# illini-robomaster/irmv_detection

Measured on AMD Instinct MI355X. Metric: end-to-end FPS (preprocess→NMS→PnP) 640×640 YOLOv8n, 1/2/4/8 MI355X, higher is better.
Workload: dtype f16

## Files before the change

irmv_detection_amd/csrc/irmv_common.hpp:

```cpp
#pragma once

#include <hip/hip_runtime.h>

#include <cstdint>
#include <cstdlib>

namespace irmv {

typedef _Float16 half_t;
typedef _Float16 half8 __attribute__((ext_vector_type(8)));
typedef _Float16 half4 __attribute__((ext_vector_type(4)));
typedef float f32x4 __attribute__((ext_vector_type(4)));

constexpr float kActScale = 1.44269504088896341f;
constexpr float kActUnscale = 0.693147180559945309f;
typedef unsigned int u32x4_t __attribute__((ext_vector_type(4)));
__device__ __forceinline__ float silu_rcp(float y) { return __builtin_amdgcn_rcpf(1.0f + __builtin_amdgcn_exp2f(-y)); }
__device__ __forceinline__ unsigned int silu_pack2(float y0, float y1)
{
    const float r0 = silu_rcp(y0), r1 = silu_rcp(y1);
    unsigned int o;
    asm("v_fma_mixlo_f16 %0, %1, %2, 0" : "=v"(o) : "v"(y0), "v"(r0));
    asm("v_fma_mixhi_f16 %0, %1, %2, 0" : "+v"(o) : "v"(y1), "v"(r1));
    return o;
}
__device__ __forceinline__ half8 silu_pack8(float y0, float y1, float y2, float y3, float y4, float y5, float y6, float y7)
{
    return __builtin_bit_cast(half8, (u32x4_t){silu_pack2(y0, y1), silu_pack2(y2, y3), silu_pack2(y4, y5), silu_pack2(y6, y7)});
}
__device__ __forceinline__ half4 silu_pack4(float y0, float y1, float y2, float y3)
{
    typedef unsigned int u32x2_t __attribute__((ext_vector_type(2)));
    return __builtin_bit_cast(half4, (u32x2_t){silu_pack2(y0, y1), silu_pack2(y2, y3)});
}
__device__ __forceinline__ void mfma_operand_fence(half4 &x) { asm volatile("s_nop 1" : "+v"(x)); }
__device__ __forceinline__ void mfma_operand_fence(half8 &x, half8 &y) { asm volatile("s_nop 1" : "+v"(x), "+v"(y)); }
__device__ __forceinline__ half_t silu_add_res(float y, float res)
{
    float p = y * silu_rcp(y);
    asm("" : "+v"(p));
    float s = p + res;
    asm("" : "+v"(s));
    return (half_t)s;
}

__device__ __forceinline__ void tile_image(int id, int tiles, int batch, int xcd, int &tile, int &image)
{
    const int full = xcd ? (batch >> 3) * 8 * tiles : 0;
    if (id < full) {
        const int j = id >> 3;
        image = (j / tiles) * 8 + (id & 7);
        tile = j % tiles;
    } else {
        const int r = id - full;
        image = (full / tiles) + r / tiles;
        tile = r % tiles;
    }
}

inline int xcd_image_order()
{
    const char *v = getenv("IRMV_XCD_IMAGES");
    return (v && v[0] == '0') ? 0 : 1;
}

inline int wres_stagger()
{
    const char *v = getenv("IRMV_WRES_STAGGER");
    return (v && v[0] == '0') ? 0 : 1;
}

constexpr int kHeadRec = 96;
constexpr int kClsOff = 64;
constexpr int kKptOff = 80;
constexpr int kCandCap = 8192;
constexpr int kMaxDetCap = 256;

struct AxisTap { int32_t i0, i1, w1, pad; };

struct PreArgs {
    const uint8_t *src;
    half_t *dst;
    const AxisTap *tx, *ty;
    int sw, sh, net, swap_rb;
    size_t src_slot_bytes;
};
void launch_preprocess(const PreArgs &a, int batch, hipStream_t s);
void launch_rotate180(const uint8_t *src, uint8_t *dst, int sw, int sh, hipStream_t s);
void launch_upload_frames(const uint8_t *src_host_mapped, uint8_t *dst, size_t bytes, int blocks, hipStream_t s);

constexpr int kBayerBandRows = 8;
struct BayerArgs {
    const uint8_t *raw;
    uint8_t *dst;
    size_t raw_slot_bytes, dst_slot_bytes;
    int W, H;
    int ry, rx;
    uint32_t gain[3];
};
void launch_demosaic(const BayerArgs &a, int batch, hipStream_t s);

struct Conv0Args {
    const half_t *x;
    half_t *y;
    const half_t *w;
    const float *b;
    int net, batch;
};
void launch_conv0(const Conv0Args &a, hipStream_t s);

constexpr int kFrontTileY = 4, kFrontTileX = 16;
constexpr int kFrontTileYDirect = 8;
constexpr int kFrontStageMax = 128 * 1024;
struct FrontArgs {
    const uint8_t *src;
    size_t src_slot_bytes;
    const AxisTap *tx, *ty;
    int vx0, vx1, vy0, vy1;
    int sw, sh, net, swap_rb;
    int fastx, fx_i0, fx_step;
    const half_t *w0;
    const float *b0;
    const half_t *w1;
    const float *b1;
    half_t *out;
    int out_ld;
    int tiles_x, tiles_y;
    int tile_y;
    int stage_bytes;
};
int front_min_stage_bytes(int tile_y = kFrontTileY);
bool front_prepare();
bool launch_front(const FrontArgs &a, int batch, hipStream_t s);

constexpr int kC2fTile = 16;
struct C2fArgs {
    const half_t *x;
    int x_ld;
    half_t *out;
    int out_ld;
    int S, tiles;
    const half_t *w_cv1, *w_m1, *w_m2, *w_cv2;
    const float *b_cv1, *b_m1, *b_m2, *b_cv2;
};
void launch_c2f2(const C2fArgs &a, int batch, hipStream_t s);

struct DwArgs {
    const half_t *x;
    int x_ld;
    half_t *y;
    int y_ld;
    const half_t *w;
    const float *b;
    int Hin, Win, Hout, Wout, C, stride;
};
void launch_dwconv3x3(const DwArgs &a, int batch, hipStream_t s);
struct ShufArgs {
    const half_t *a, *b;
    int a_ld, b_ld;
    half_t *out;
    int out_ld, bc;
    size_t pixels;
};
void launch_shuffle_cat(const ShufArgs &a, hipStream_t s);

struct ConvSeg {
    const half_t *p;
    int ld;
    int C;
    int shift;
};

constexpr int kC2f32TileH = 8, kC2f32TileW = 16;
struct C2f32Args {
    ConvSeg s0, s1;
    int cin1;
    half_t *cat;
    int cat_ld, prev_coff;
    half_t *out;
    int out_ld;
    int H, W, tiles_x, tiles_y;
    const half_t *w_cv1, *w_m1, *w_m2, *w_cv2;
    const float *b_cv1, *b_m1, *b_m2, *b_cv2;
};
size_t c2f32_lds_bytes(int mode);
bool launch_c2f32(int mode, bool shortcut, const C2f32Args &a, int batch, hipStream_t s);

constexpr int kBneckTile = 8;
struct BneckArgs {
    const half_t *yin;
    int yin_ld;
    half_t *ynext;
    int ynext_ld;
    const half_t *cat;
    int cat_ld;
    half_t *out;
    int out_ld;
    int H, W, tiles_x, tiles_y;
    const half_t *w_m1, *w_m2;
    const float *b_m1, *b_m2;
    const half_t *w_cv2;
    const float *b_cv2;
};
size_t bneck64_lds_bytes(int mode, int ks2);
bool launch_bneck64(int mode, int ks2, bool shortcut, const BneckArgs &a, int batch, hipStream_t s);

constexpr int kKpt3Tile = 10;
struct Kpt3Args {
    const half_t *x;
    int x_ld;
    int H, W, tiles_x, tiles_y;
    const half_t *w1;
    const float *b1;
    const half_t *w2;
    const float *b2;
    const half_t *w3;
    const float *b3;
    float *out;
    int out_ld;
};
bool kpt3_eligible(int cin);
bool launch_kpt3(const Kpt3Args &a, int cin, int batch, hipStream_t s);

struct ConvArgs {
    ConvSeg s0, s1;
    int Hin, Win;
    int Hout, Wout;
    int M;
    int Cin;
    const half_t *w;
    const float *bias;
    void *out;
    int out_ld;
    const half_t *res;
    int res_ld;
    int cout_pad;
    int ksteps;
    int pair;
    const half_t *w2;
    const float *bias2;
    float *out2;
    int out2_ld, n2;
    unsigned long long *scan_keys;
    int *scan_counts;
    float scan_thr;
    int scan_nc, scan_abase, scan_key_cap;
};

constexpr int kMultiMax = 6;
struct LdsMember {
    ConvArgs a;
    const half_t *wl;
    int tiles_x, tiles_y, twc_log2, patch_bytes, batch, tile2d;
    int gx, gy;
};
struct LdsMultiArgs {
    int n;
    int start[kMultiMax + 1];
    LdsMember m[kMultiMax];
};
struct DirectMultiArgs {
    int n;
    int start[kMultiMax + 1], gx[kMultiMax], gy[kMultiMax];
    ConvArgs a[kMultiMax];
};

struct ConvCfg {
    int ks, stride, mt, nt; bool cin16; int act; bool out_f32; bool lds; int ipw;
    bool deep;
    bool ct;
    bool pw;
    bool pf2;
    bool pf4;
    bool w8;
    int cm;
    bool wr;
    bool pp;
};
bool launch_conv(const ConvCfg &cfg, const ConvArgs &a, hipStream_t s);
const char *conv_cfg_name(const ConvCfg &cfg, char *buf, int n);
bool conv_pw_eligible(const ConvCfg &cfg, const ConvArgs &a);
bool launch_conv_lds_multi(int nt, const ConvArgs *a, const half_t *const *wl, int n, int batch, hipStream_t s);
bool launch_conv_direct_multi(const ConvCfg &cfg, const ConvArgs *a, int n, hipStream_t s);
bool launch_conv_k16(const ConvArgs &a, hipStream_t s);
bool launch_conv_pw(const ConvCfg &cfg, const ConvArgs &a, hipStream_t s);
size_t conv_pw_lds_bytes(const ConvArgs &a, int nbw);
size_t conv_lds_bytes(const ConvArgs &a, int stride, int mt, int nt, int *patch_rows_max, bool w8 = false);
size_t conv_wres_bytes(const ConvArgs &a, int stride, bool pp);
int conv_wres_tiles(const ConvArgs &a, int stride, bool pp);
bool launch_conv_wres(int ipw, const ConvArgs &a, const half_t *wl, int batch, hipStream_t s, bool pp);
bool launch_conv_lds(int stride, int mt, int nt, int ipw, const ConvArgs &a, const half_t *wl, int batch, hipStream_t s, int pf2 = 0, int cm = 0, bool w8 = false);

void launch_sppf_pool(half_t *buf, int batch, int H, int W, int C, hipStream_t s);

struct DevDet {
    float box_net[4];
    float xyxy[4];
    float score;
    int32_t cls, anchor, pnp_ok;
    float kpts_net[8];
    float kpts[8];
    double rvec[3], tvec[3], quat[4];
    int32_t armor_valid;
    int32_t armor_size;
    int32_t n_lights;
    int32_t pad_;
};
struct DevFrameOut { int32_t num_dets, n_candidates, overflow, pad; };

struct PnpConst {
    double fx, fy, cx, cy, k1, k2, p1, p2, k3;
    double hy[2], hz[2];
};

struct PostArgs {
    const float *head_all;
    int slots_total, first;
    float *boxes;
    unsigned long long *keys;
    int key_cap;
    DevDet *dets;
    DevFrameOut *fout;
    int net, A, nc, nk;
    float logit_thr, iou_thr;
    int max_det, pre_nms_cap;
    float scale_x, scale_y, off_x, off_y;
    int armor_size;
    const PnpConst *pnp;
    long long *dbg;
    int keys_only;
    int prefilter;
    int classwalk;
    int *counts;
};
void launch_nms_pnp(const PostArgs &a, int batch, hipStream_t s);
constexpr int kScanBlocks = 16;
void launch_scan_decode(const PostArgs &a, int batch, hipStream_t s);
constexpr int kLightLdsPoints = 256;
constexpr int kLightLdsImage = 40 * 1024;
constexpr int kLightMaxContours = 1024;

struct LightArgs {
    const uint8_t *frames;
    size_t frame_bytes;
    int cols, rows, rotate180;
    DevDet *dets;
    int max_det;
    const int *num_dets;
    int num_dets_stride, n_boxes;
    const float *boxes;
    signed char *labels;
    size_t label_pool;
    short *points;
    int points_cap;
    short *hulls;
    int binary_threshold;
    float light_min_ratio, light_max_ratio, light_max_angle;
    double min_small_cd, max_small_cd, min_large_cd, max_large_cd;
    const PnpConst *pnp;
    int pnp_armor_size;
};
void launch_light_extract(const LightArgs &a, int n_boxes_max, int batch, hipStream_t s);

void launch_pnp_only(const PnpConst &c, const float *pts, int n, int armor_size, double *rvec, double *tvec,
                     int32_t *ok, hipStream_t s);

}
```

irmv_detection_amd/csrc/k_c2f.hip:

```cpp
#include "irmv_common.hpp"

#include <cstdlib>
#include <mutex>

namespace irmv {

namespace {
constexpr int T = kC2fTile;
constexpr int XW = T + 4, XN = XW * XW;
constexpr int TW = T + 2, TN = TW * TW;
constexpr int HP = 32;

__device__ __forceinline__ f32x4 bias4(const float *b) { return (f32x4){b[0], b[1], b[2], b[3]}; }

typedef unsigned int u32x4 __attribute__((ext_vector_type(4)));
__device__ __forceinline__ u32x4 ld16(const half_t *p) { return *reinterpret_cast<const u32x4 *>(p); }
__device__ __forceinline__ u32x4 keep_if(bool c, u32x4 v) { return c ? v : (u32x4){0u, 0u, 0u, 0u}; }
__device__ __forceinline__ half8 as_h8(u32x4 v) { return __builtin_bit_cast(half8, v); }

template <int RH, int RW>
__device__ __forceinline__ bool region_tile_px(int t, int r, int &ly, int &lx)
{
    constexpr int LC = RW - 16;
    static_assert(LC == 2 || LC == 4, "16 columns + a power of two");
    if (t < RH) { ly = t; lx = r; return true; }
    const int q = (t - RH) * 16 + r;
    const bool ok = q < LC * RH;
    ly = ok ? q / LC : 0;
    lx = ok ? 16 + (q & (LC - 1)) : 0;
    return ok;
}
}

__global__ __launch_bounds__(256) void c2f2_kernel(C2fArgs a, int batch, int xcd)
{
    __shared__ __attribute__((aligned(16))) uint8_t s_y0[T * T * HP];
    __shared__ __attribute__((aligned(16))) uint8_t s_y1[XN * HP];
    __shared__ __attribute__((aligned(16))) uint8_t s_t[TN * HP];
    __shared__ __attribute__((aligned(16))) uint8_t s_y2[T * T * HP];
    const int tid = threadIdx.x, lane = tid & 63, wave = tid >> 6;
    const int g = lane >> 4, r = lane & 15;
    int tile_id, b;
    tile_image(blockIdx.x, a.tiles * a.tiles, batch, xcd, tile_id, b);
    const int tyi = tile_id / a.tiles, txi = tile_id - tyi * a.tiles;
    const int oy0 = tyi * T, ox0 = txi * T;
    const int S = a.S;
    const half8 zero8 = (half8){0, 0, 0, 0, 0, 0, 0, 0};

    const half8 *w;
    w = reinterpret_cast<const half8 *>(a.w_cv1) + lane;
    const half8 Wc1[2] = {w[0], w[64]};
    half8 Wm1[5], Wm2[5];
    w = reinterpret_cast<const half8 *>(a.w_m1) + lane;
#pragma unroll
    for (int ks = 0; ks < 5; ks++) Wm1[ks] = w[ks * 64];
    float bias_c1[8];
#pragma unroll
    for (int i = 0; i < 8; i++) bias_c1[i] = a.b_cv1[g * 8 + i];
    __shared__ float s_bias[16 + 16 + 32];
    if (tid < 16) { s_bias[tid] = a.b_m1[tid]; s_bias[16 + tid] = a.b_m2[tid]; }
    else if (tid < 48) s_bias[16 + tid] = a.b_cv2[tid - 16];

    {
        const float (&bias)[8] = bias_c1;
        constexpr int NROWT = XW / 4, NCOLT = (XN / 16 - XW + 3) / 4;
        static_assert(XW % 4 == 0 && XW - 16 == 4 && NCOLT == 2, "20 row tiles + 5 column tiles");
        const char *xbase = reinterpret_cast<const char *>(a.x);
        const uint32_t img = (uint32_t)b * (uint32_t)(S * S);
        auto px_off = [&](int gy, int gx) -> uint32_t {
            const int gyc = gy < 0 ? 0 : (gy >= S ? S - 1 : gy), gxc = gx < 0 ? 0 : (gx >= S ? S - 1 : gx);
            return ((img + (uint32_t)(gyc * S + gxc)) * (uint32_t)a.x_ld + 8u * g) * 2u;
        };
        const int gx_r = ox0 - 2 + r;
        const bool in_x = (unsigned)gx_r < (unsigned)S;
        int ly_c[NCOLT], lx_c[NCOLT];
        bool has_c[NCOLT];
#pragma unroll
        for (int k = 0; k < NCOLT; k++) {
            const int tc = wave + 4 * k, q = tc * 16 + r;
            has_c[k] = tc < XN / 16 - XW;
            ly_c[k] = has_c[k] ? q >> 2 : 0;
            lx_c[k] = 16 + (q & 3);
        }
        u32x4 Bq[NROWT + NCOLT];
#pragma unroll
        for (int i = 0; i < NROWT; i++) Bq[i] = *reinterpret_cast<const u32x4 *>(xbase + px_off(oy0 - 2 + wave + 4 * i, gx_r));
#pragma unroll
        for (int k = 0; k < NCOLT; k++) Bq[NROWT + k] = *reinterpret_cast<const u32x4 *>(xbase + px_off(oy0 - 2 + ly_c[k], ox0 - 2 + lx_c[k]));
        auto run_tile = [&](u32x4 bq, int ly, int lx, bool inside) {
            const int m = ly * XW + lx;
            f32x4 acc0 = bias4(bias), acc1 = bias4(bias + 4);
            acc0 = __builtin_amdgcn_mfma_f32_16x16x32_f16(Wc1[0], as_h8(bq), acc0, 0, 0, 0);
            acc1 = __builtin_amdgcn_mfma_f32_16x16x32_f16(Wc1[1], as_h8(bq), acc1, 0, 0, 0);
            half8 o = zero8;
            if (inside) o = silu_pack8(acc0[0], acc0[1], acc0[2], acc0[3], acc1[0], acc1[1], acc1[2], acc1[3]);
            if (g >= 2) {
                *reinterpret_cast<half8 *>(s_y1 + m * HP + (g - 2) * 16) = o;
            } else if ((unsigned)(ly - 2) < (unsigned)T && (unsigned)(lx - 2) < (unsigned)T) {
                *reinterpret_cast<half8 *>(s_y0 + ((ly - 2) * T + (lx - 2)) * HP + g * 16) = o;
            }
        };
#pragma unroll
        for (int i = 0; i < NROWT; i++) {
            const int t = wave + 4 * i, gy = oy0 - 2 + t;
            run_tile(Bq[i], t, r, in_x && (unsigned)gy < (unsigned)S);
        }
#pragma unroll
        for (int k = 0; k < NCOLT; k++) {
            if (!has_c[k]) break;
            const int gy = oy0 - 2 + ly_c[k], gx = ox0 - 2 + lx_c[k];
            run_tile(Bq[NROWT + k], ly_c[k], lx_c[k], (unsigned)gy < (unsigned)S && (unsigned)gx < (unsigned)S);
        }
    }
    __syncthreads();

    w = reinterpret_cast<const half8 *>(a.w_m2) + lane;
#pragma unroll
    for (int ks = 0; ks < 5; ks++) Wm2[ks] = w[ks * 64];
    w = reinterpret_cast<const half8 *>(a.w_cv2) + lane;
    const half8 Wc2[2][2] = {{w[0], w[64]}, {w[128], w[192]}};

    {
        float bias[4];
#pragma unroll
        for (int i = 0; i < 4; i++) bias[i] = s_bias[g * 4 + i];
        int toff[5];
#pragma unroll
        for (int ks = 0; ks < 5; ks++) {
            const int tap = 2 * ks + (g >> 1), kh = tap / 3, kw = tap - kh * 3;
            toff[ks] = tap < 9 ? (kh * XW + kw) * HP + 16 * (g & 1) : -1;
        }
        for (int t = wave; t < (TN + 15) / 16; t += 4) {
            int ly, lx;
            const bool mv = region_tile_px<TW, TW>(t, r, ly, lx);
            const int m = ly * TW + lx;
            const uint8_t *base = s_y1 + (ly * XW + lx) * HP;
            f32x4 acc = bias4(bias);
#pragma unroll
            for (int ks = 0; ks < 5; ks++) {
                half8 B = zero8;
                if (toff[ks] >= 0) B = *reinterpret_cast<const half8 *>(base + toff[ks]);
                acc = __builtin_amdgcn_mfma_f32_16x16x32_f16(Wm1[ks], B, acc, 0, 0, 0);
            }
            if (mv) {
                const int gy = oy0 - 1 + ly, gx = ox0 - 1 + lx;
                half4 o = (half4){0, 0, 0, 0};
                if ((unsigned)gy < (unsigned)S && (unsigned)gx < (unsigned)S) o = silu_pack4(acc[0], acc[1], acc[2], acc[3]);
                *reinterpret_cast<half4 *>(s_t + m * HP + g * 8) = o;
            }
        }
    }
    __syncthreads();

    {
        float bias[4];
#pragma unroll
        for (int i = 0; i < 4; i++) bias[i] = s_bias[16 + g * 4 + i];
        int toff[5];
#pragma unroll
        for (int ks = 0; ks < 5; ks++) {
            const int tap = 2 * ks + (g >> 1), kh = tap / 3, kw = tap - kh * 3;
            toff[ks] = tap < 9 ? (kh * TW + kw) * HP + 16 * (g & 1) : -1;
        }
        for (int t = wave; t < T * T / 16; t += 4) {
            const int m = t * 16 + r;
            const int ly = m / T, lx = m - ly * T;
            const uint8_t *base = s_t + (ly * TW + lx) * HP;
            f32x4 acc = bias4(bias);
#pragma unroll
            for (int ks = 0; ks < 5; ks++) {
                half8 B = zero8;
                if (toff[ks] >= 0) B = *reinterpret_cast<const half8 *>(base + toff[ks]);
                acc = __builtin_amdgcn_mfma_f32_16x16x32_f16(Wm2[ks], B, acc, 0, 0, 0);
            }
            const half4 rv = *reinterpret_cast<const half4 *>(s_y1 + ((ly + 2) * XW + lx + 2) * HP + g * 8);
            half4 o;
#pragma unroll
            for (int i = 0; i < 4; i++) o[i] = silu_add_res(acc[i], (float)rv[i]);
            *reinterpret_cast<half4 *>(s_y2 + m * HP + g * 8) = o;
        }
    }
    __syncthreads();

    {
        float bias[8];
#pragma unroll
        for (int i = 0; i < 8; i++) bias[i] = s_bias[32 + g * 8 + i];
        half_t *out = a.out + (size_t)b * S * S * a.out_ld;
        for (int t = wave; t < T * T / 16; t += 4) {
            const int m = t * 16 + r;
            const int ly = m / T, lx = m - ly * T;
            const half8 B0 = g < 2 ? *reinterpret_cast<const half8 *>(s_y0 + m * HP + g * 16)
                                   : *reinterpret_cast<const half8 *>(s_y1 + ((ly + 2) * XW + lx + 2) * HP + (g - 2) * 16);
            half8 B1 = zero8;
            if (g < 2) B1 = *reinterpret_cast<const half8 *>(s_y2 + m * HP + g * 16);
            f32x4 acc0 = bias4(bias), acc1 = bias4(bias + 4);
            acc0 = __builtin_amdgcn_mfma_f32_16x16x32_f16(Wc2[0][0], B0, acc0, 0, 0, 0);
            acc1 = __builtin_amdgcn_mfma_f32_16x16x32_f16(Wc2[1][0], B0, acc1, 0, 0, 0);
            acc0 = __builtin_amdgcn_mfma_f32_16x16x32_f16(Wc2[0][1], B1, acc0, 0, 0, 0);
            acc1 = __builtin_amdgcn_mfma_f32_16x16x32_f16(Wc2[1][1], B1, acc1, 0, 0, 0);
            const int gy = oy0 + ly, gx = ox0 + lx;
            if (gy < S && gx < S) {
                const half8 o = silu_pack8(acc0[0], acc0[1], acc0[2], acc0[3], acc1[0], acc1[1], acc1[2], acc1[3]);
                *reinterpret_cast<half8 *>(out + ((size_t)gy * S + gx) * a.out_ld + g * 8) = o;
            }
        }
    }
}

static int c2f_xcd_order() { return xcd_image_order(); }

void launch_c2f2(const C2fArgs &a, int batch, hipStream_t s)
{
    hipLaunchKernelGGL(c2f2_kernel, dim3(a.tiles * a.tiles * batch), dim3(256), 0, s, a, batch, c2f_xcd_order());
}


namespace {
constexpr int FH = kC2f32TileH, FW = kC2f32TileW;
constexpr int R1H = FH + 4, R1W = FW + 4, R1N = R1H * R1W;
constexpr int R2H = FH + 2, R2W = FW + 2, R2N = R2H * R2W;
constexpr int R3N = FH * FW;
constexpr int PS = 96;
static_assert(R1N % 16 == 0 && R3N % 16 == 0, "tile regions are whole MFMA tiles");
}

template <int MODE, int KS1, bool SHORTCUT>
__global__ __launch_bounds__(256) void c2f32_kernel(C2f32Args a, int batch, int xcd)
{
    extern __shared__ __attribute__((aligned(16))) uint8_t smem[];
    uint8_t *s_in = smem;
    uint8_t *s_t = s_in + R1N * PS;
    uint8_t *s_yn = s_t + R2N * PS;
    uint8_t *s_y0 = s_yn + R3N * PS;
    const int tid = threadIdx.x, lane = tid & 63, wave = tid >> 6;
    const int g = lane >> 4, r = lane & 15;
    int tile_id, b;
    tile_image(blockIdx.x, a.tiles_x * a.tiles_y, batch, xcd, tile_id, b);
    const int tyi = tile_id / a.tiles_x, txi = tile_id - tyi * a.tiles_x;
    const int oy0 = tyi * FH, ox0 = txi * FW;
    const int H = a.H, W = a.W;
    const half8 zero8 = (half8){0, 0, 0, 0, 0, 0, 0, 0};
    half_t *cat = a.cat + (size_t)b * H * W * a.cat_ld;
    __shared__ float s_bias[32 + 32 + 64];
    if (tid < 32) { s_bias[tid] = a.b_m1[tid]; s_bias[32 + tid] = a.b_m2[tid]; }
    if (MODE != 1 && tid < 64) s_bias[64 + tid] = a.b_cv2[tid];

    u32x4 Y01[2][2];
    static_assert(R3N / 16 == 8, "two output tiles per wave");
    if constexpr (MODE != 2) {
        half8 W1[4][KS1];
        {
            const half8 *w = reinterpret_cast<const half8 *>(a.w_cv1) + lane;
#pragma unroll
            for (int nt = 0; nt < 4; nt++)
#pragma unroll
                for (int ks = 0; ks < KS1; ks++) W1[nt][ks] = w[(size_t)(nt * KS1 + ks) * 64];
        }
        float bias[16];
#pragma unroll
        for (int u = 0; u < 2; u++)
#pragma unroll
            for (int i = 0; i < 8; i++) bias[u * 8 + i] = a.b_cv1[u * 32 + g * 8 + i];
        const int H0 = H >> a.s0.shift, W0 = W >> a.s0.shift, H1 = H >> a.s1.shift, W1s = W >> a.s1.shift;
        constexpr int NT1 = R1N / 16, NROWT = R1H / 4, NCOLT = NT1 - R1H;
        static_assert(R1H % 4 == 0 && NCOLT >= 0 && NCOLT <= 4 && R1W - 16 == 4, "three row tiles per wave, at most one column tile");
        const char *base0 = reinterpret_cast<const char *>(a.s0.p), *base1 = reinterpret_cast<const char *>(a.s1.p - a.s0.C);
        const uint32_t img0 = (uint32_t)b * (uint32_t)(H0 * W0), img1 = (uint32_t)b * (uint32_t)(H1 * W1s);
        auto px_off = [&](int gyc, int gxc, uint32_t &o0, uint32_t &o1) {
            o0 = ((img0 + (uint32_t)((gyc >> a.s0.shift) * W0 + (gxc >> a.s0.shift))) * (uint32_t)a.s0.ld + 8u * g) * 2u;
            o1 = ((img1 + (uint32_t)((gyc >> a.s1.shift) * W1s + (gxc >> a.s1.shift))) * (uint32_t)a.s1.ld + 8u * g) * 2u;
        };
        auto issue = [&](uint32_t o0, uint32_t o1, u32x4 (&B)[KS1]) {
#pragma unroll
            for (int ks = 0; ks < KS1; ks++) {
                const bool seg0 = ks * 32 < a.s0.C;
                B[ks] = *reinterpret_cast<const u32x4 *>((seg0 ? base0 : base1) + ((seg0 ? o0 : o1) + (uint32_t)(ks * 64)));
            }
        };
        const int gx_r = ox0 - 2 + r;
        const bool in_x = (unsigned)gx_r < (unsigned)W;
        const int gxc_r = gx_r < 0 ? 0 : (gx_r >= W ? W - 1 : gx_r);
        auto row_off = [&](int t, uint32_t &o0, uint32_t &o1) {
            const int gy = oy0 - 2 + t, gyc = gy < 0 ? 0 : (gy >= H ? H - 1 : gy);
            px_off(gyc, gxc_r, o0, o1);
        };
        const int q_c = 16 * wave + r, ly_c = q_c >> 2, lx_c = 16 + (q_c & 3);
        const bool has_col = wave < NCOLT;
        auto run_tile = [&](const u32x4 (&Bq)[KS1], int ly, int lx, bool inside, bool want_y0) {
            const int m = ly * R1W + lx;
            const int gy = oy0 - 2 + ly, gx = ox0 - 2 + lx;
            f32x4 acc[4];
#pragma unroll
            for (int nt = 0; nt < 4; nt++) acc[nt] = bias4(bias + (nt >> 1) * 8 + (nt & 1) * 4);
            if (want_y0) {
#pragma unroll
                for (int ks = 0; ks < KS1; ks++)
#pragma unroll
                    for (int nt = 0; nt < 4; nt++) acc[nt] = __builtin_amdgcn_mfma_f32_16x16x32_f16(W1[nt][ks], as_h8(Bq[ks]), acc[nt], 0, 0, 0);
            } else {
#pragma unroll
                for (int ks = 0; ks < KS1; ks++)
#pragma unroll
                    for (int nt = 2; nt < 4; nt++) acc[nt] = __builtin_amdgcn_mfma_f32_16x16x32_f16(W1[nt][ks], as_h8(Bq[ks]), acc[nt], 0, 0, 0);
            }
            half8 o[2];
#pragma unroll
            for (int u = 0; u < 2; u++) {
                o[u] = zero8;
                if (inside && (u == 1 || want_y0)) {
                    o[u] = silu_pack8(acc[2 * u][0], acc[2 * u][1], acc[2 * u][2], acc[2 * u][3], acc[2 * u + 1][0], acc[2 * u + 1][1], acc[2 * u + 1][2], acc[2 * u + 1][3]);
                }
            }
            *reinterpret_cast<half8 *>(s_in + m * PS + g * 16) = o[1];
            const int cy = ly - 2, cx = lx - 2;
            if (inside && (unsigned)cy < (unsigned)FH && (unsigned)cx < (unsigned)FW) {
                if constexpr (MODE == 0) {
                    *reinterpret_cast<half8 *>(s_y0 + (cy * FW + cx) * PS + g * 16) = o[0];
                } else {
                    half_t *qd = cat + ((size_t)gy * W + gx) * a.cat_ld + g * 8;
                    *reinterpret_cast<half8 *>(qd) = o[0];
                    *reinterpret_cast<half8 *>(qd + 32) = o[1];
                }
            }
        };
        u32x4 Bn[KS1], Bc[KS1];
        {
            uint32_t o0, o1;
            row_off(wave, o0, o1);
            issue(o0, o1, Bn);
        }
#pragma unroll
        for (int i = 0; i < NROWT; i++) {
            const int t = wave + 4 * i;
#pragma unroll
            for (int ks = 0; ks < KS1; ks++) Bc[ks] = Bn[ks];
            {
                uint32_t o0, o1;
                if (i + 1 < NROWT) {
                    row_off(t + 4, o0, o1);
                    issue(o0, o1, Bn);
                } else if (has_col) {
                    const int gy = oy0 - 2 + ly_c, gx = ox0 - 2 + lx_c;
                    px_off(gy < 0 ? 0 : (gy >= H ? H - 1 : gy), gx < 0 ? 0 : (gx >= W ? W - 1 : gx), o0, o1);
                    issue(o0, o1, Bn);
                }
            }
            const int gy = oy0 - 2 + t;
            run_tile(Bc, t, r, in_x && (unsigned)gy < (unsigned)H, t >= 2 && t < R1H - 2);
        }
        if (has_col) {
            const int gy = oy0 - 2 + ly_c, gx = ox0 - 2 + lx_c;
            run_tile(Bn, ly_c, lx_c, (unsigned)gy < (unsigned)H && (unsigned)gx < (unsigned)W, true);
        }
    } else {
#pragma unroll
        for (int i = 0; i < 2; i++) {
            const int m = (wave + 4 * i) * 16 + r;
            const int ly = m / FW, lx = m - ly * FW;
            const int gy = oy0 + ly, gx = ox0 + lx;
            const bool in = gy < H && gx < W;
            const half_t *q = cat + ((size_t)(in ? gy : 0) * W + (in ? gx : 0)) * a.cat_ld + g * 8;
            Y01[i][0] = ld16(q);
            Y01[i][1] = ld16(q + 32);
        }
        const half_t *src = cat + a.prev_coff;
        constexpr int NP = (R1N * 4 + 255) / 256;
        u32x4 v[NP];
#pragma unroll
        for (int i = 0; i < NP; i++) {
            const int e = tid + i * 256;
            const int m = e >> 2, q = e & 3;
            const int ly = m / R1W, lx = m - ly * R1W;
            const int gy = oy0 - 2 + ly, gx = ox0 - 2 + lx;
            const bool in = e < R1N * 4 && (unsigned)gy < (unsigned)H && (unsigned)gx < (unsigned)W;
            v[i] = ld16(src + ((size_t)(in ? gy : 0) * W + (in ? gx : 0)) * a.cat_ld + q * 8);
        }
#pragma unroll
        for (int i = 0; i < NP; i++) {
            const int e = tid + i * 256;
            const int m = e >> 2;
            const int ly = m / R1W, lx = m - ly * R1W;
            const int gy = oy0 - 2 + ly, gx = ox0 - 2 + lx;
            if (e < R1N * 4) *reinterpret_cast<u32x4 *>(s_in + m * PS + (e & 3) * 16) = keep_if((unsigned)gy < (unsigned)H && (unsigned)gx < (unsigned)W, v[i]);
        }
    }
    __syncthreads();

    {
        half8 Wm[2][9];
        const half8 *w = reinterpret_cast<const half8 *>(a.w_m1) + lane;
#pragma unroll
        for (int nt = 0; nt < 2; nt++)
#pragma unroll
            for (int tap = 0; tap < 9; tap++) Wm[nt][tap] = w[(size_t)(nt * 9 + tap) * 64];
        float bias[8];
#pragma unroll
        for (int i = 0; i < 8; i++) bias[i] = s_bias[g * 8 + i];
        for (int t = wave; t < (R2N + 15) / 16; t += 4) {
            int ly, lx;
            const bool mv = region_tile_px<R2H, R2W>(t, r, ly, lx);
            const int m = ly * R2W + lx;
            const uint8_t *base = s_in + (ly * R1W + lx) * PS + g * 16;
            f32x4 acc0 = bias4(bias), acc1 = bias4(bias + 4);
#pragma unroll
            for (int tap = 0; tap < 9; tap++) {
                const half8 B = *reinterpret_cast<const half8 *>(base + ((tap / 3) * R1W + (tap % 3)) * PS);
                acc0 = __builtin_amdgcn_mfma_f32_16x16x32_f16(Wm[0][tap], B, acc0, 0, 0, 0);
                acc1 = __builtin_amdgcn_mfma_f32_16x16x32_f16(Wm[1][tap], B, acc1, 0, 0, 0);
            }
            if (mv) {
                const int gy = oy0 - 1 + ly, gx = ox0 - 1 + lx;
                half8 o = zero8;
                if ((unsigned)gy < (unsigned)H && (unsigned)gx < (unsigned)W) o = silu_pack8(acc0[0], acc0[1], acc0[2], acc0[3], acc1[0], acc1[1], acc1[2], acc1[3]);
                *reinterpret_cast<half8 *>(s_t + m * PS + g * 16) = o;
            }
        }
    }
    __syncthreads();

    {
        half8 Wm[2][9];
        const half8 *w = reinterpret_cast<const half8 *>(a.w_m2) + lane;
#pragma unroll
        for (int nt = 0; nt < 2; nt++)
#pragma unroll
            for (int tap = 0; tap < 9; tap++) Wm[nt][tap] = w[(size_t)(nt * 9 + tap) * 64];
        float bias[8];
#pragma unroll
        for (int i = 0; i < 8; i++) bias[i] = s_bias[32 + g * 8 + i];
        for (int t = wave; t < R3N / 16; t += 4) {
            const int m = t * 16 + r;
            const int ly = m / FW, lx = m - ly * FW;
            const uint8_t *base = s_t + (ly * R2W + lx) * PS + g * 16;
            f32x4 acc0 = bias4(bias), acc1 = bias4(bias + 4);
#pragma unroll
            for (int tap = 0; tap < 9; tap++) {
                const half8 B = *reinterpret_cast<const half8 *>(base + ((tap / 3) * R2W + (tap % 3)) * PS);
                acc0 = __builtin_amdgcn_mfma_f32_16x16x32_f16(Wm[0][tap], B, acc0, 0, 0, 0);
                acc1 = __builtin_amdgcn_mfma_f32_16x16x32_f16(Wm[1][tap], B, acc1, 0, 0, 0);
            }
            half8 o;
            half8 rv = zero8;
            if constexpr (SHORTCUT) rv = *reinterpret_cast<const half8 *>(s_in + ((ly + 2) * R1W + lx + 2) * PS + g * 16);
            if constexpr (SHORTCUT) {
#pragma unroll
                for (int i = 0; i < 8; i++) o[i] = silu_add_res(i < 4 ? acc0[i] : acc1[i - 4], (float)rv[i]);
            } else {
                o = silu_pack8(acc0[0], acc0[1], acc0[2], acc0[3], acc1[0], acc1[1], acc1[2], acc1[3]);
            }
            if constexpr (MODE == 1) {
                const int gy = oy0 + ly, gx = ox0 + lx;
                if (gy < H && gx < W) *reinterpret_cast<half8 *>(cat + ((size_t)gy * W + gx) * a.cat_ld + 64 + g * 8) = o;
            } else {
                *reinterpret_cast<half8 *>(s_yn + m * PS + g * 16) = o;
            }
        }
    }
    if constexpr (MODE == 1) return;
    __syncthreads();

    {
        constexpr int KS2 = MODE == 0 ? 3 : 4;
        half8 W2[4][KS2];
        const half8 *w = reinterpret_cast<const half8 *>(a.w_cv2) + lane;
#pragma unroll
        for (int nt = 0; nt < 4; nt++)
#pragma unroll
            for (int ks = 0; ks < KS2; ks++) W2[nt][ks] = w[(size_t)(nt * KS2 + ks) * 64];
        float bias[16];
#pragma unroll
        for (int u = 0; u < 2; u++)
#pragma unroll
            for (int i = 0; i < 8; i++) bias[u * 8 + i] = s_bias[64 + u * 32 + g * 8 + i];
        half_t *out = a.out + (size_t)b * H * W * a.out_ld;
        for (int t = wave; t < R3N / 16; t += 4) {
            const int m = t * 16 + r;
            const int ly = m / FW, lx = m - ly * FW;
            const int gy = oy0 + ly, gx = ox0 + lx;
            const bool inside = gy < H && gx < W;
            half8 B[KS2];
            if constexpr (MODE == 0) {
                B[0] = *reinterpret_cast<const half8 *>(s_y0 + m * PS + g * 16);
                B[1] = *reinterpret_cast<const half8 *>(s_in + ((ly + 2) * R1W + lx + 2) * PS + g * 16);
                B[2] = *reinterpret_cast<const half8 *>(s_yn + m * PS + g * 16);
            } else {
                B[0] = as_h8(keep_if(inside, Y01[(t - wave) >> 2][0]));
                B[1] = as_h8(keep_if(inside, Y01[(t - wave) >> 2][1]));
                B[2] = *reinterpret_cast<const half8 *>(s_in + ((ly + 2) * R1W + lx + 2) * PS + g * 16);
                B[3] = *reinterpret_cast<const half8 *>(s_yn + m * PS + g * 16);
            }
            f32x4 acc[4];
#pragma unroll
            for (int nt = 0; nt < 4; nt++) acc[nt] = bias4(bias + (nt >> 1) * 8 + (nt & 1) * 4);
#pragma unroll
            for (int ks = 0; ks < KS2; ks++)
#pragma unroll
                for (int nt = 0; nt < 4; nt++) acc[nt] = __builtin_amdgcn_mfma_f32_16x16x32_f16(W2[nt][ks], B[ks], acc[nt], 0, 0, 0);
            if (inside) {
#pragma unroll
                for (int u = 0; u < 2; u++) {
                    const half8 o = silu_pack8(acc[2 * u][0], acc[2 * u][1], acc[2 * u][2], acc[2 * u][3], acc[2 * u + 1][0], acc[2 * u + 1][1], acc[2 * u + 1][2], acc[2 * u + 1][3]);
                    *reinterpret_cast<half8 *>(out + ((size_t)gy * W + gx) * a.out_ld + u * 32 + g * 8) = o;
                }
            }
        }
    }
}

static std::mutex g_c2f_attr_mu;

size_t c2f32_lds_bytes(int mode) { return (size_t)(R1N + R2N + (mode == 1 ? 0 : R3N) + (mode == 0 ? R3N : 0)) * PS; }

bool launch_c2f32(int mode, bool shortcut, const C2f32Args &a, int batch, hipStream_t s)
{
    const int ks1 = a.cin1 / 32;
    const dim3 grid(a.tiles_x * a.tiles_y * batch), block(256);
    const int xcd = c2f_xcd_order();
    const size_t lds = c2f32_lds_bytes(mode);
#define IRMV_C2F32(MODE_, KS_, SC_)                                                                               \
    if (mode == MODE_ && (MODE_ == 2 || ks1 == KS_) && shortcut == SC_) {                                          \
        static unsigned long long attr_done = 0;                                                                   \
        int dev = 0; (void)hipGetDevice(&dev);                                                                     \
        {                                    \
            std::lock_guard<std::mutex> lk(g_c2f_attr_mu);                                                         \
            if (!(attr_done & (1ull << (dev & 63)))) {                                                             \
                (void)hipFuncSetAttribute(reinterpret_cast<const void *>(c2f32_kernel<MODE_, KS_, SC_>), hipFuncAttributeMaxDynamicSharedMemorySize, 96 * 1024); \
                attr_done |= 1ull << (dev & 63);                                                                   \
            }                                                                                                      \
        }                                                                                                          \
        hipLaunchKernelGGL((c2f32_kernel<MODE_, KS_, SC_>), grid, block, lds, s, a, batch, xcd);                   \
        return true;                                                                                               \
    }
    IRMV_C2F32(0, 2, true) IRMV_C2F32(0, 2, false) IRMV_C2F32(0, 4, false) IRMV_C2F32(0, 6, false) IRMV_C2F32(0, 6, true) IRMV_C2F32(0, 4, true)
    IRMV_C2F32(1, 2, true) IRMV_C2F32(1, 2, false) IRMV_C2F32(1, 4, true) IRMV_C2F32(1, 6, true)
    IRMV_C2F32(2, 1, true) IRMV_C2F32(2, 1, false)
#undef IRMV_C2F32
    return false;
}

}
```

Before: 60240.

## Shrink c2f32 LDS footprint and stage cv1 weights in LDS for occupancy

```diff
diff --git a/irmv_detection_amd/csrc/irmv_common.hpp b/irmv_detection_amd/csrc/irmv_common.hpp
--- a/irmv_detection_amd/csrc/irmv_common.hpp
+++ b/irmv_detection_amd/csrc/irmv_common.hpp
@@ -183,7 +183,7 @@
     const half_t *w_cv1, *w_m1, *w_m2, *w_cv2;
     const float *b_cv1, *b_m1, *b_m2, *b_cv2;
 };
-size_t c2f32_lds_bytes(int mode);
+size_t c2f32_lds_bytes(int mode, int ks1);
 bool launch_c2f32(int mode, bool shortcut, const C2f32Args &a, int batch, hipStream_t s);
 
 constexpr int kBneckTile = 8;
diff --git a/irmv_detection_amd/csrc/k_c2f.hip b/irmv_detection_amd/csrc/k_c2f.hip
--- a/irmv_detection_amd/csrc/k_c2f.hip
+++ b/irmv_detection_amd/csrc/k_c2f.hip
@@ -1,7 +1,9 @@
 #include "irmv_common.hpp"
 
+#include <cstdio>
 #include <cstdlib>
 #include <mutex>
+#include <type_traits>
 
 namespace irmv {
 
@@ -221,18 +223,31 @@
 constexpr int R1H = FH + 4, R1W = FW + 4, R1N = R1H * R1W;
 constexpr int R2H = FH + 2, R2W = FW + 2, R2N = R2H * R2W;
 constexpr int R3N = FH * FW;
-constexpr int PS = 96;
+constexpr int PS = 64;
 static_assert(R1N % 16 == 0 && R3N % 16 == 0, "tile regions are whole MFMA tiles");
+
+__device__ __forceinline__ int plane_off(int p, int s) { return p * PS + ((s ^ ((p >> 1) & 2)) << 4); }
+
+__host__ __device__ constexpr bool c2f32_w1_lds(int mode, int ks1) { return mode == 0 || (mode == 1 && ks1 > 2); }
+__host__ __device__ constexpr int c2f32_w1_off(int mode) { return (R1N + (mode == 0 ? R3N : 0)) * PS; }
+__host__ __device__ constexpr int c2f32_lds(int mode, int ks1)
+{
+    const int planes = c2f32_w1_off(mode) + (R2N + (mode == 1 ? 0 : R3N)) * PS;
+    const int w1 = c2f32_w1_lds(mode, ks1) ? c2f32_w1_off(mode) + ks1 * 4 * 64 * 16 : 0;
+    return planes > w1 ? planes : w1;
+}
+static_assert(c2f32_lds(0, 6) + 512 <= 160 * 1024 / 3 && c2f32_lds(1, 2) + 512 <= 160 * 1024 / 4 && c2f32_lds(2, 1) + 512 <= 160 * 1024 / 4,
+              "LDS for three (AB) / four (A, B) workgroups per CU");
 }
 
 template <int MODE, int KS1, bool SHORTCUT>
-__global__ __launch_bounds__(256) void c2f32_kernel(C2f32Args a, int batch, int xcd)
+__global__ __launch_bounds__(256) __attribute__((amdgpu_waves_per_eu(MODE == 0 ? 3 : 4))) void c2f32_kernel(C2f32Args a, int batch, int xcd)
 {
     extern __shared__ __attribute__((aligned(16))) uint8_t smem[];
     uint8_t *s_in = smem;
-    uint8_t *s_t = s_in + R1N * PS;
+    uint8_t *s_y0 = s_in + R1N * PS;
+    uint8_t *s_t = smem + c2f32_w1_off(MODE);
     uint8_t *s_yn = s_t + R2N * PS;
-    uint8_t *s_y0 = s_yn + R3N * PS;
     const int tid = threadIdx.x, lane = tid & 63, wave = tid >> 6;
     const int g = lane >> 4, r = lane & 15;
     int tile_id, b;
@@ -249,14 +264,24 @@
     u32x4 Y01[2][2];
     static_assert(R3N / 16 == 8, "two output tiles per wave");
     if constexpr (MODE != 2) {
-        half8 W1[4][KS1];
-        {
+        constexpr bool W1_LDS = c2f32_w1_lds(MODE, KS1);
+        const half8 *s_w1 = reinterpret_cast<const half8 *>(s_t);
+        u32x4 wst[W1_LDS ? KS1 : 1];
+        half8 W1r[W1_LDS ? 1 : 4][W1_LDS ? 1 : KS1];
+        if constexpr (W1_LDS) {
+#pragma unroll
+            for (int i = 0; i < KS1; i++) wst[i] = ld16(a.w_cv1 + (size_t)(tid + 256 * i) * 8);
+        } else {
             const half8 *w = reinterpret_cast<const half8 *>(a.w_cv1) + lane;
 #pragma unroll
             for (int nt = 0; nt < 4; nt++)
 #pragma unroll
-                for (int ks = 0; ks < KS1; ks++) W1[nt][ks] = w[(size_t)(nt * KS1 + ks) * 64];
-        }
+                for (int ks = 0; ks < KS1; ks++) W1r[nt][ks] = w[(size_t)(nt * KS1 + ks) * 64];
+        }
+        auto w1 = [&](int nt, int ks) -> half8 {
+            if constexpr (W1_LDS) return s_w1[(nt * KS1 + ks) * 64 + lane];
+            else return W1r[nt][ks];
+        };
         float bias[16];
 #pragma unroll
         for (int u = 0; u < 2; u++)
@@ -293,17 +318,23 @@
             f32x4 acc[4];
 #pragma unroll
             for (int nt = 0; nt < 4; nt++) acc[nt] = bias4(bias + (nt >> 1) * 8 + (nt & 1) * 4);
-            if (want_y0) {
-#pragma unroll
-                for (int ks = 0; ks < KS1; ks++)
-#pragma unroll
-                    for (int nt = 0; nt < 4; nt++) acc[nt] = __builtin_amdgcn_mfma_f32_16x16x32_f16(W1[nt][ks], as_h8(Bq[ks]), acc[nt], 0, 0, 0);
-            } else {
-#pragma unroll
-                for (int ks = 0; ks < KS1; ks++)
-#pragma unroll
-                    for (int nt = 2; nt < 4; nt++) acc[nt] = __builtin_amdgcn_mfma_f32_16x16x32_f16(W1[nt][ks], as_h8(Bq[ks]), acc[nt], 0, 0, 0);
-            }
+            auto mfmas = [&](auto nt0) {
+                constexpr int NT0 = decltype(nt0)::value;
+                half8 A[2][4];
+#pragma unroll
+                for (int nt = NT0; nt < 4; nt++) A[0][nt] = w1(nt, 0);
+#pragma unroll
+                for (int ks = 0; ks < KS1; ks++) {
+                    if (ks + 1 < KS1) {
+#pragma unroll
+                        for (int nt = NT0; nt < 4; nt++) A[(ks + 1) & 1][nt] = w1(nt, ks + 1);
+                    }
+#pragma unroll
+                    for (int nt = NT0; nt < 4; nt++) acc[nt] = __builtin_amdgcn_mfma_f32_16x16x32_f16(A[ks & 1][nt], as_h8(Bq[ks]), acc[nt], 0, 0, 0);
+                }
+            };
+            if (want_y0) mfmas(std::integral_constant<int, 0>{});
+            else mfmas(std::integral_constant<int, 2>{});
             half8 o[2];
 #pragma unroll
             for (int u = 0; u < 2; u++) {
@@ -312,11 +343,11 @@
                     o[u] = silu_pack8(acc[2 * u][0], acc[2 * u][1], acc[2 * u][2], acc[2 * u][3], acc[2 * u + 1][0], acc[2 * u + 1][1], acc[2 * u + 1][2], acc[2 * u + 1][3]);
                 }
             }
-            *reinterpret_cast<half8 *>(s_in + m * PS + g * 16) = o[1];
+            *reinterpret_cast<half8 *>(s_in + plane_off(m, g)) = o[1];
             const int cy = ly - 2, cx = lx - 2;
             if (inside && (unsigned)cy < (unsigned)FH && (unsigned)cx < (unsigned)FW) {
                 if constexpr (MODE == 0) {
-                    *reinterpret_cast<half8 *>(s_y0 + (cy * FW + cx) * PS + g * 16) = o[0];
+                    *reinterpret_cast<half8 *>(s_y0 + plane_off(cy * FW + cx, g)) = o[0];
                 } else {
                     half_t *qd = cat + ((size_t)gy * W + gx) * a.cat_ld + g * 8;
                     *reinterpret_cast<half8 *>(qd) = o[0];
@@ -329,6 +360,11 @@
             uint32_t o0, o1;
             row_off(wave, o0, o1);
             issue(o0, o1, Bn);
+        }
+        if constexpr (W1_LDS) {
+#pragma unroll
+            for (int i = 0; i < KS1; i++) *reinterpret_cast<u32x4 *>(s_t + (tid + 256 * i) * 16) = wst[i];
+            __syncthreads();
         }
 #pragma unroll
         for (int i = 0; i < NROWT; i++) {
@@ -354,6 +390,100 @@
             run_tile(Bn, ly_c, lx_c, (unsigned)gy < (unsigned)H && (unsigned)gx < (unsigned)W, true);
         }
     } else {
+        const half_t *src = cat + a.prev_coff;
+        constexpr int NP = (R1N * 4 + 255) / 256;
+        u32x4 v[NP];
+#pragma unroll
+        for (int i = 0; i < NP; i++) {
+            const int e = tid + i * 256;
+            const int m = e >> 2, q = e & 3;
+            const int ly = m / R1W, lx = m - ly * R1W;
+            const int gy = oy0 - 2 + ly, gx = ox0 - 2 + lx;
+            const bool in = e < R1N * 4 && (unsigned)gy < (unsigned)H && (unsigned)gx < (unsigned)W;
+            v[i] = ld16(src + ((size_t)(in ? gy : 0) * W + (in ? gx : 0)) * a.cat_ld + q * 8);
+        }
+#pragma unroll
+        for (int i = 0; i < NP; i++) {
+            const int e = tid + i * 256;
+            const int m = e >> 2;
+            const int ly = m / R1W, lx = m - ly * R1W;
+            const int gy = oy0 - 2 + ly, gx = ox0 - 2 + lx;
+            if (e < R1N * 4) *reinterpret_cast<u32x4 *>(s_in + plane_off(m, e & 3)) = keep_if((unsigned)gy < (unsigned)H && (unsigned)gx < (unsigned)W, v[i]);
+        }
+    }
+    __syncthreads();
+
+    {
+        half8 Wm[2][9];
+        const half8 *w = reinterpret_cast<const half8 *>(a.w_m1) + lane;
+#pragma unroll
+        for (int nt = 0; nt < 2; nt++)
+#pragma unroll
+            for (int tap = 0; tap < 9; tap++) Wm[nt][tap] = w[(size_t)(nt * 9 + tap) * 64];
+        float bias[8];
+#pragma unroll
+        for (int i = 0; i < 8; i++) bias[i] = s_bias[g * 8 + i];
+        for (int t = wave; t < (R2N + 15) / 16; t += 4) {
+            int ly, lx;
+            const bool mv = region_tile_px<R2H, R2W>(t, r, ly, lx);
+            const int m = ly * R2W + lx, p = ly * R1W + lx;
+            f32x4 acc0 = bias4(bias), acc1 = bias4(bias + 4);
+#pragma unroll
+            for (int tap = 0; tap < 9; tap++) {
+                const half8 B = *reinterpret_cast<const half8 *>(s_in + plane_off(p + (tap / 3) * R1W + tap % 3, g));
+                acc0 = __builtin_amdgcn_mfma_f32_16x16x32_f16(Wm[0][tap], B, acc0, 0, 0, 0);
+                acc1 = __builtin_amdgcn_mfma_f32_16x16x32_f16(Wm[1][tap], B, acc1, 0, 0, 0);
+            }
+            if (mv) {
+                const int gy = oy0 - 1 + ly, gx = ox0 - 1 + lx;
+                half8 o = zero8;
+                if ((unsigned)gy < (unsigned)H && (unsigned)gx < (unsigned)W) o = silu_pack8(acc0[0], acc0[1], acc0[2], acc0[3], acc1[0], acc1[1], acc1[2], acc1[3]);
+                *reinterpret_cast<half8 *>(s_t + plane_off(m, g)) = o;
+            }
+        }
+    }
+    __syncthreads();
+
+    {
+        half8 Wm[2][9];
+        const half8 *w = reinterpret_cast<const half8 *>(a.w_m2) + lane;
+#pragma unroll
+        for (int nt = 0; nt < 2; nt++)
+#pragma unroll
+            for (int tap = 0; tap < 9; tap++) Wm[nt][tap] = w[(size_t)(nt * 9 + tap) * 64];
+        float bias[8];
+#pragma unroll
+        for (int i = 0; i < 8; i++) bias[i] = s_bias[32 + g * 8 + i];
+        for (int t = wave; t < R3N / 16; t += 4) {
+            const int m = t * 16 + r;
+            const int ly = m / FW, lx = m - ly * FW;
+            const int p = ly * R2W + lx;
+            f32x4 acc0 = bias4(bias), acc1 = bias4(bias + 4);
+#pragma unroll
+            for (int tap = 0; tap < 9; tap++) {
+                const half8 B = *reinterpret_cast<const half8 *>(s_t + plane_off(p + (tap / 3) * R2W + tap % 3, g));
+                acc0 = __builtin_amdgcn_mfma_f32_16x16x32_f16(Wm[0][tap], B, acc0, 0, 0, 0);
+                acc1 = __builtin_amdgcn_mfma_f32_16x16x32_f16(Wm[1][tap], B, acc1, 0, 0, 0);
+            }
+            half8 o;
+            half8 rv = zero8;
+            if constexpr (SHORTCUT) rv = *reinterpret_cast<const half8 *>(s_in + plane_off((ly + 2) * R1W + lx + 2, g));
+            if constexpr (SHORTCUT) {
+#pragma unroll
+                for (int i = 0; i < 8; i++) o[i] = silu_add_res(i < 4 ? acc0[i] : acc1[i - 4], (float)rv[i]);
+            } else {
+                o = silu_pack8(acc0[0], acc0[1], acc0[2], acc0[3], acc1[0], acc1[1], acc1[2], acc1[3]);
+            }
+            if constexpr (MODE == 1) {
+                const int gy = oy0 + ly, gx = ox0 + lx;
+                if (gy < H && gx < W) *reinterpret_cast<half8 *>(cat + ((size_t)gy * W + gx) * a.cat_ld + 64 + g * 8) = o;
+            } else {
+                *reinterpret_cast<half8 *>(s_yn + plane_off(m, g)) = o;
+            }
+        }
+    }
+    if constexpr (MODE == 1) return;
+    if constexpr (MODE == 2) {
 #pragma unroll
         for (int i = 0; i < 2; i++) {
             const int m = (wave + 4 * i) * 16 + r;
@@ -364,100 +494,7 @@
             Y01[i][0] = ld16(q);
             Y01[i][1] = ld16(q + 32);
         }
-        const half_t *src = cat + a.prev_coff;
-        constexpr int NP = (R1N * 4 + 255) / 256;
-        u32x4 v[NP];
-#pragma unroll
-        for (int i = 0; i < NP; i++) {
-            const int e = tid + i * 256;
-            const int m = e >> 2, q = e & 3;
-            const int ly = m / R1W, lx = m - ly * R1W;
-            const int gy = oy0 - 2 + ly, gx = ox0 - 2 + lx;
-            const bool in = e < R1N * 4 && (unsigned)gy < (unsigned)H && (unsigned)gx < (unsigned)W;
-            v[i] = ld16(src + ((size_t)(in ? gy : 0) * W + (in ? gx : 0)) * a.cat_ld + q * 8);
-        }
-#pragma unroll
-        for (int i = 0; i < NP; i++) {
-            const int e = tid + i * 256;
-            const int m = e >> 2;
-            const int ly = m / R1W, lx = m - ly * R1W;
-            const int gy = oy0 - 2 + ly, gx = ox0 - 2 + lx;
-            if (e < R1N * 4) *reinterpret_cast<u32x4 *>(s_in + m * PS + (e & 3) * 16) = keep_if((unsigned)gy < (unsigned)H && (unsigned)gx < (unsigned)W, v[i]);
-        }
-    }
-    __syncthreads();
-
-    {
-        half8 Wm[2][9];
-        const half8 *w = reinterpret_cast<const half8 *>(a.w_m1) + lane;
-#pragma unroll
-        for (int nt = 0; nt < 2; nt++)
-#pragma unroll
-            for (int tap = 0; tap < 9; tap++) Wm[nt][tap] = w[(size_t)(nt * 9 + tap) * 64];
-        float bias[8];
-#pragma unroll
-        for (int i = 0; i < 8; i++) bias[i] = s_bias[g * 8 + i];
-        for (int t = wave; t < (R2N + 15) / 16; t += 4) {
-            int ly, lx;
-            const bool mv = region_tile_px<R2H, R2W>(t, r, ly, lx);
-            const int m = ly * R2W + lx;
-            const uint8_t *base = s_in + (ly * R1W + lx) * PS + g * 16;
-            f32x4 acc0 = bias4(bias), acc1 = bias4(bias + 4);
-#pragma unroll
-            for (int tap = 0; tap < 9; tap++) {
-                const half8 B = *reinterpret_cast<const half8 *>(base + ((tap / 3) * R1W + (tap % 3)) * PS);
-                acc0 = __builtin_amdgcn_mfma_f32_16x16x32_f16(Wm[0][tap], B, acc0, 0, 0, 0);
-                acc1 = __builtin_amdgcn_mfma_f32_16x16x32_f16(Wm[1][tap], B, acc1, 0, 0, 0);
-            }
-            if (mv) {
-                const int gy = oy0 - 1 + ly, gx = ox0 - 1 + lx;
-                half8 o = zero8;
-                if ((unsigned)gy < (unsigned)H && (unsigned)gx < (unsigned)W) o = silu_pack8(acc0[0], acc0[1], acc0[2], acc0[3], acc1[0], acc1[1], acc1[2], acc1[3]);
-                *reinterpret_cast<half8 *>(s_t + m * PS + g * 16) = o;
-            }
-        }
-    }
-    __syncthreads();
-
-    {
-        half8 Wm[2][9];
-        const half8 *w = reinterpret_cast<const half8 *>(a.w_m2) + lane;
-#pragma unroll
-        for (int nt = 0; nt < 2; nt++)
-#pragma unroll
-            for (int tap = 0; tap < 9; tap++) Wm[nt][tap] = w[(size_t)(nt * 9 + tap) * 64];
-        float bias[8];
-#pragma unroll
-        for (int i = 0; i < 8; i++) bias[i] = s_bias[32 + g * 8 + i];
-        for (int t = wave; t < R3N / 16; t += 4) {
-            const int m = t * 16 + r;
-            const int ly = m / FW, lx = m - ly * FW;
-            const uint8_t *base = s_t + (ly * R2W + lx) * PS + g * 16;
-            f32x4 acc0 = bias4(bias), acc1 = bias4(bias + 4);
-#pragma unroll
-            for (int tap = 0; tap < 9; tap++) {
-                const half8 B = *reinterpret_cast<const half8 *>(base + ((tap / 3) * R2W + (tap % 3)) * PS);
-                acc0 = __builtin_amdgcn_mfma_f32_16x16x32_f16(Wm[0][tap], B, acc0, 0, 0, 0);
-                acc1 = __builtin_amdgcn_mfma_f32_16x16x32_f16(Wm[1][tap], B, acc1, 0, 0, 0);
-            }
-            half8 o;
-            half8 rv = zero8;
-            if constexpr (SHORTCUT) rv = *reinterpret_cast<const half8 *>(s_in + ((ly + 2) * R1W + lx + 2) * PS + g * 16);
-            if constexpr (SHORTCUT) {
-#pragma unroll
-                for (int i = 0; i < 8; i++) o[i] = silu_add_res(i < 4 ? acc0[i] : acc1[i - 4], (float)rv[i]);
-            } else {
-                o = silu_pack8(acc0[0], acc0[1], acc0[2], acc0[3], acc1[0], acc1[1], acc1[2], acc1[3]);
-            }
-            if constexpr (MODE == 1) {
-                const int gy = oy0 + ly, gx = ox0 + lx;
-                if (gy < H && gx < W) *reinterpret_cast<half8 *>(cat + ((size_t)gy * W + gx) * a.cat_ld + 64 + g * 8) = o;
-            } else {
-                *reinterpret_cast<half8 *>(s_yn + m * PS + g * 16) = o;
-            }
-        }
-    }
-    if constexpr (MODE == 1) return;
+    }
     __syncthreads();
 
     {
@@ -473,7 +510,7 @@
         for (int u = 0; u < 2; u++)
 #pragma unroll
             for (int i = 0; i < 8; i++) bias[u * 8 + i] = s_bias[64 + u * 32 + g * 8 + i];
-        half_t *out = a.out + (size_t)b * H * W * a.out_ld;
+        char *out = reinterpret_cast<char *>(a.out + (size_t)b * H * W * a.out_ld);
         for (int t = wave; t < R3N / 16; t += 4) {
             const int m = t * 16 + r;
             const int ly = m / FW, lx = m - ly * FW;
@@ -481,14 +518,14 @@
             const bool inside = gy < H && gx < W;
             half8 B[KS2];
             if constexpr (MODE == 0) {
-                B[0] = *reinterpret_cast<const half8 *>(s_y0 + m * PS + g * 16);
-                B[1] = *reinterpret_cast<const half8 *>(s_in + ((ly + 2) * R1W + lx + 2) * PS + g * 16);
-                B[2] = *reinterpret_cast<const half8 *>(s_yn + m * PS + g * 16);
+                B[0] = *reinterpret_cast<const half8 *>(s_y0 + plane_off(m, g));
+                B[1] = *reinterpret_cast<const half8 *>(s_in + plane_off((ly + 2) * R1W + lx + 2, g));
+                B[2] = *reinterpret_cast<const half8 *>(s_yn + plane_off(m, g));
             } else {
                 B[0] = as_h8(keep_if(inside, Y01[(t - wave) >> 2][0]));
                 B[1] = as_h8(keep_if(inside, Y01[(t - wave) >> 2][1]));
-                B[2] = *reinterpret_cast<const half8 *>(s_in + ((ly + 2) * R1W + lx + 2) * PS + g * 16);
-                B[3] = *reinterpret_cast<const half8 *>(s_yn + m * PS + g * 16);
+                B[2] = *reinterpret_cast<const half8 *>(s_in + plane_off((ly + 2) * R1W + lx + 2, g));
+                B[3] = *reinterpret_cast<const half8 *>(s_yn + plane_off(m, g));
             }
             f32x4 acc[4];
 #pragma unroll
@@ -501,7 +538,7 @@
 #pragma unroll
                 for (int u = 0; u < 2; u++) {
                     const half8 o = silu_pack8(acc[2 * u][0], acc[2 * u][1], acc[2 * u][2], acc[2 * u][3], acc[2 * u + 1][0], acc[2 * u + 1][1], acc[2 * u + 1][2], acc[2 * u + 1][3]);
-                    *reinterpret_cast<half8 *>(out + ((size_t)gy * W + gx) * a.out_ld + u * 32 + g * 8) = o;
+                    *reinterpret_cast<half8 *>(out + (uint32_t)(((gy * W + gx) * a.out_ld + u * 32 + g * 8) * 2)) = o;
                 }
             }
         }
@@ -510,22 +547,28 @@
 
 static std::mutex g_c2f_attr_mu;
 
-size_t c2f32_lds_bytes(int mode) { return (size_t)(R1N + R2N + (mode == 1 ? 0 : R3N) + (mode == 0 ? R3N : 0)) * PS; }
+size_t c2f32_lds_bytes(int mode, int ks1) { return (size_t)c2f32_lds(mode, ks1); }
+
+static bool log_occupancy() { static const bool on = getenv("IRMV_LOG_OCCUPANCY") != nullptr; return on; }
 
 bool launch_c2f32(int mode, bool shortcut, const C2f32Args &a, int batch, hipStream_t s)
 {
     const int ks1 = a.cin1 / 32;
     const dim3 grid(a.tiles_x * a.tiles_y * batch), block(256);
     const int xcd = c2f_xcd_order();
-    const size_t lds = c2f32_lds_bytes(mode);
 #define IRMV_C2F32(MODE_, KS_, SC_)                                                                               \
     if (mode == MODE_ && (MODE_ == 2 || ks1 == KS_) && shortcut == SC_) {                                          \
+        constexpr int lds = c2f32_lds(MODE_, KS_);                                                                 \
+        const void *fn = reinterpret_cast<const void *>(c2f32_kernel<MODE_, KS_, SC_>);                            \
         static unsigned long long attr_done = 0;                                                                   \
         int dev = 0; (void)hipGetDevice(&dev);                                                                     \
         {                                    \
             std::lock_guard<std::mutex> lk(g_c2f_attr_mu);                                                         \
             if (!(attr_done & (1ull << (dev & 63)))) {                                                             \
-                (void)hipFuncSetAttribute(reinterpret_cast<const void *>(c2f32_kernel<MODE_, KS_, SC_>), hipFuncAttributeMaxDynamicSharedMemorySize, 96 * 1024); \
+                (void)hipFuncSetAttribute(fn, hipFuncAttributeMaxDynamicSharedMemorySize, lds);                    \
+                int nb = 0;                                                                                        \
+                if (log_occupancy() && hipOccupancyMaxActiveBlocksPerMultiprocessor(&nb, fn, 256, lds) == hipSuccess) \
+                    fprintf(stderr, "irmv: c2f32_kernel<%d, %d, %d> on device %d: %d B LDS, %d workgroups per CU\n", MODE_, KS_, (int)SC_, dev, lds, nb); \
                 attr_done |= 1ull << (dev & 63);                                                                   \
             }                                                                                                      \
         }                                                                                                          \
```

Measured after the change: 60400 (median of 6 runs). About the same (+0.3%).
